# kujason/monopsr

Hardware: AMD Instinct MI355X
Metric: instance-crops/sec (fwd+Chamfer) (higher is better)
Workload: dtype f32; 1 GPU; BASELINE cfg3: batch=256/GPU synthetic 48x48 crops -> ResNet-101 trunk(block3, os4) + squash/map-decoder/xyz + heads fwd, + 1024-pt nn_distance Chamfer fwd/bwd; batch_per_gpu=256, global_batch=256, points=1024, streams_per_gpu=1

## Files before the change

### monopsr_amd/csrc/image_ops.hip

```cpp
#include "common.h"

#pragma clang fp contract(off)

namespace {

template <int V>
struct Vec;
template <>
struct Vec<4> {
    using type = float4;
};
template <>
struct Vec<1> {
    using type = float;
};

__device__ __forceinline__ float4 lerp4(float4 a, float4 b, float t)
{
    return make_float4(a.x + (b.x - a.x) * t, a.y + (b.y - a.y) * t, a.z + (b.z - a.z) * t, a.w + (b.w - a.w) * t);
}
__device__ __forceinline__ float lerp4(float a, float b, float t) { return a + (b - a) * t; }
__device__ __forceinline__ float4 splat(float v, float4) { return make_float4(v, v, v, v); }
__device__ __forceinline__ float splat(float v, float) { return v; }
__device__ __forceinline__ float4 vmax(float4 a, float4 b)
{
    return make_float4(fmaxf(a.x, b.x), fmaxf(a.y, b.y), fmaxf(a.z, b.z), fmaxf(a.w, b.w));
}
__device__ __forceinline__ float vmax(float a, float b) { return fmaxf(a, b); }

template <int V>
__global__ __launch_bounds__(256) void crop_and_resize_kernel(const float *__restrict__ image, int H, int W, int C,
                                                              const float *__restrict__ boxes,
                                                              const int *__restrict__ box_ind, int nimg, int ch,
                                                              int cw, float extrap, float *__restrict__ out,
                                                              long long total)
{
    using T = typename Vec<V>::type;
    const int cv = C / V;
    for (long long i = (long long)blockIdx.x * blockDim.x + threadIdx.x; i < total;
         i += (long long)gridDim.x * blockDim.x) {
        const int c = (int)(i % cv);
        long long r = i / cv;
        const int x = (int)(r % cw);
        r /= cw;
        const int y = (int)(r % ch);
        const int bi = (int)(r / ch);
        const float y1 = boxes[4 * bi], x1 = boxes[4 * bi + 1], y2 = boxes[4 * bi + 2], x2 = boxes[4 * bi + 3];
        const int img = box_ind ? box_ind[bi] : 0;
        T res = splat(extrap, T());
        const float hs = ch > 1 ? (y2 - y1) * (float)(H - 1) / (float)(ch - 1) : 0.f;
        const float ws = cw > 1 ? (x2 - x1) * (float)(W - 1) / (float)(cw - 1) : 0.f;
        const float in_y = ch > 1 ? y1 * (float)(H - 1) + (float)y * hs : 0.5f * (y1 + y2) * (float)(H - 1);
        const float in_x = cw > 1 ? x1 * (float)(W - 1) + (float)x * ws : 0.5f * (x1 + x2) * (float)(W - 1);
        if (img >= 0 && img < nimg && !(in_y < 0.f) && !(in_y > (float)(H - 1)) && !(in_x < 0.f) &&
            !(in_x > (float)(W - 1)) && in_y == in_y && in_x == in_x) {
            const int top = (int)floorf(in_y), bot = (int)ceilf(in_y);
            const int left = (int)floorf(in_x), right = (int)ceilf(in_x);
            const float yl = in_y - (float)top, xl = in_x - (float)left;
            const T *base = reinterpret_cast<const T *>(image + (size_t)img * H * W * C);
            const T tl = base[((size_t)top * W + left) * cv + c], tr = base[((size_t)top * W + right) * cv + c];
            const T bl = base[((size_t)bot * W + left) * cv + c], br = base[((size_t)bot * W + right) * cv + c];
            res = lerp4(lerp4(tl, tr, xl), lerp4(bl, br, xl), yl);
        }
        reinterpret_cast<T *>(out)[i] = res;
    }
}

template <int V>
__global__ __launch_bounds__(256) void resize_bilinear_kernel(const float *__restrict__ in, int H, int W, int C,
                                                              int OH, int OW, float hscale, float wscale,
                                                              float *__restrict__ out, long long total)
{
    using T = typename Vec<V>::type;
    const int cv = C / V;
    for (long long i = (long long)blockIdx.x * blockDim.x + threadIdx.x; i < total;
         i += (long long)gridDim.x * blockDim.x) {
        const int c = (int)(i % cv);
        long long r = i / cv;
        const int ox = (int)(r % OW);
        r /= OW;
        const int oy = (int)(r % OH);
        const int b = (int)(r / OH);
        const float sy = (float)oy * hscale, sx = (float)ox * wscale;
        const int y0 = (int)floorf(sy), x0 = (int)floorf(sx);
        const int y1 = min(y0 + 1, H - 1), x1 = min(x0 + 1, W - 1);
        const float yl = sy - (float)y0, xl = sx - (float)x0;
        const T *base = reinterpret_cast<const T *>(in + (size_t)b * H * W * C);
        const T tl = base[((size_t)y0 * W + x0) * cv + c], tr = base[((size_t)y0 * W + x1) * cv + c];
        const T bl = base[((size_t)y1 * W + x0) * cv + c], br = base[((size_t)y1 * W + x1) * cv + c];
        reinterpret_cast<T *>(out)[i] = lerp4(lerp4(tl, tr, xl), lerp4(bl, br, xl), yl);
    }
}

template <int V>
__global__ __launch_bounds__(256) void resize_bilinear_rows_kernel(const float *__restrict__ in, int H, int W, int C,
                                                                   int OH, int OW, float hscale, float wscale,
                                                                   float *__restrict__ out)
{
    using T = typename Vec<V>::type;
    const unsigned cv = (unsigned)(C / V);
    const unsigned idx = blockIdx.x * 256u + threadIdx.x;
    if (idx >= (unsigned)OW * cv) return;
    const unsigned ox = idx / cv, c = idx - ox * cv;
    const int oy = blockIdx.y, b = blockIdx.z;
    const float sy = (float)oy * hscale, sx = (float)ox * wscale;
    const int y0 = (int)floorf(sy), x0 = (int)floorf(sx);
    const int y1 = min(y0 + 1, H - 1), x1 = min(x0 + 1, W - 1);
    const float yl = sy - (float)y0, xl = sx - (float)x0;
    const T *base = reinterpret_cast<const T *>(in + (size_t)b * H * W * C);
    const T tl = base[((size_t)y0 * W + x0) * cv + c], tr = base[((size_t)y0 * W + x1) * cv + c];
    const T bl = base[((size_t)y1 * W + x0) * cv + c], br = base[((size_t)y1 * W + x1) * cv + c];
    reinterpret_cast<T *>(out)[((size_t)b * OH + oy) * OW * cv + idx] = lerp4(lerp4(tl, tr, xl), lerp4(bl, br, xl), yl);
}

__global__ __launch_bounds__(256) void resize_bilinear_c8out_kernel(const float *__restrict__ in, int H, int W, int C,
                                                                    int OH, int OW, float hscale, float wscale,
                                                                    float *__restrict__ out)
{
    const unsigned planes = (unsigned)C / 8u;
    const unsigned idx = blockIdx.x * 256u + threadIdx.x;
    if (idx >= planes * (unsigned)OW) return;
    const unsigned plane = idx / (unsigned)OW, ox = idx - plane * (unsigned)OW;
    const int oy = blockIdx.y, b = blockIdx.z;
    const float sy = (float)oy * hscale, sx = (float)ox * wscale;
    const int y0 = (int)floorf(sy), x0 = (int)floorf(sx);
    const int y1 = min(y0 + 1, H - 1), x1 = min(x0 + 1, W - 1);
    const float yl = sy - (float)y0, xl = sx - (float)x0;
    const float4 *base = reinterpret_cast<const float4 *>(in + (size_t)b * H * W * C) + plane * 2;
    const size_t cv = (size_t)C / 4;
    float4 *dst = reinterpret_cast<float4 *>(out + ((((size_t)b * planes + plane) * OH + oy) * OW + ox) * 8);
#pragma unroll
    for (int h = 0; h < 2; ++h) {
        const float4 tl = base[((size_t)y0 * W + x0) * cv + h], tr = base[((size_t)y0 * W + x1) * cv + h];
        const float4 bl = base[((size_t)y1 * W + x0) * cv + h], br = base[((size_t)y1 * W + x1) * cv + h];
        dst[h] = lerp4(lerp4(tl, tr, xl), lerp4(bl, br, xl), yl);
    }
}

constexpr int kResizeLdsMaxRows = 16, kResizeLdsIters = 4;
__global__ __launch_bounds__(256) void resize_bilinear_c8out_lds_kernel(const float *__restrict__ in, int H, int W, int C,
                                                                        int OH, int OW, int RO, float hscale,
                                                                        float wscale, float *__restrict__ out)
{
    extern __shared__ __attribute__((aligned(16))) float4 rows[];
    const int plane = blockIdx.x, oy0 = blockIdx.y * RO, b = blockIdx.z;
    const int planes = C / 8;
    const int oy_last = min(oy0 + RO, OH) - 1;
    const int y_lo = (int)floorf((float)oy0 * hscale);
    const int y_hi = min((int)floorf((float)oy_last * hscale) + 1, H - 1);
    const int nrows = y_hi - y_lo + 1;
    const float4 *base = reinterpret_cast<const float4 *>(in + (size_t)b * H * W * C) + plane * 2;
    const size_t cv = (size_t)C / 4;
    for (int i = threadIdx.x; i < nrows * W * 2; i += 256) {
        const int h = i & 1, px = i >> 1;
        const int r = px / W, x = px - r * W;
        rows[i] = base[((size_t)(y_lo + r) * W + x) * cv + h];
    }
    __syncthreads();
    const int rpi = 256 / OW;
    const int r = threadIdx.x / OW, ox = threadIdx.x - r * OW;
    if (r >= rpi) return;
    const float sx = (float)ox * wscale;
    const int x0 = (int)floorf(sx), x1 = min(x0 + 1, W - 1);
    const float xl = sx - (float)x0;
    for (int oy = oy0 + r; oy <= oy_last; oy += rpi) {
        const float sy = (float)oy * hscale;
        const int y0 = (int)floorf(sy), y1 = min(y0 + 1, H - 1);
        const float yl = sy - (float)y0;
        float4 *dst = reinterpret_cast<float4 *>(out + ((((size_t)b * planes + plane) * OH + oy) * OW + ox) * 8);
#pragma unroll
        for (int h = 0; h < 2; ++h) {
            const float4 tl = rows[((y0 - y_lo) * W + x0) * 2 + h], tr = rows[((y0 - y_lo) * W + x1) * 2 + h];
            const float4 bl = rows[((y1 - y_lo) * W + x0) * 2 + h], br = rows[((y1 - y_lo) * W + x1) * 2 + h];
            dst[h] = lerp4(lerp4(tl, tr, xl), lerp4(bl, br, xl), yl);
        }
    }
}

template <int V>
__global__ __launch_bounds__(256) void max_pool_kernel(const float *__restrict__ in, int H, int W, int C, int OH,
                                                       int OW, int k, int s, int pad_top, int pad_left,
                                                       float *__restrict__ out, long long total)
{
    using T = typename Vec<V>::type;
    const int cv = C / V;
    for (long long i = (long long)blockIdx.x * blockDim.x + threadIdx.x; i < total;
         i += (long long)gridDim.x * blockDim.x) {
        const int c = (int)(i % cv);
        long long r = i / cv;
        const int ox = (int)(r % OW);
        r /= OW;
        const int oy = (int)(r % OH);
        const int b = (int)(r / OH);
        const T *base = reinterpret_cast<const T *>(in + (size_t)b * H * W * C);
        T best = splat(-__builtin_inff(), T());
        for (int ky = 0; ky < k; ++ky) {
            const int y = oy * s - pad_top + ky;
            if (y < 0 || y >= H) continue;
            for (int kx = 0; kx < k; ++kx) {
                const int x = ox * s - pad_left + kx;
                if (x < 0 || x >= W) continue;
                best = vmax(best, base[((size_t)y * W + x) * cv + c]);
            }
        }
        reinterpret_cast<T *>(out)[i] = best;
    }
}

__global__ __launch_bounds__(256) void im2col_root_kernel(const float *__restrict__ x, int H, int W, int OH, int OW,
                                                          int kpad, float *__restrict__ cols, long long total)
{
    for (long long i = (long long)blockIdx.x * blockDim.x + threadIdx.x; i < total;
         i += (long long)gridDim.x * blockDim.x) {
        const int j = (int)(i % kpad);
        long long r = i / kpad;
        const int ox = (int)(r % OW);
        r /= OW;
        const int oy = (int)(r % OH);
        const int b = (int)(r / OH);
        float v = 0.f;
        if (j < 147) {
            const int c = j % 3, t = j / 3;
            const int kx = t % 7, ky = t / 7;
            const int yy = oy * 2 + ky - 3, xx = ox * 2 + kx - 3;
            if (yy >= 0 && yy < H && xx >= 0 && xx < W) v = x[(((size_t)b * H + yy) * W + xx) * 3 + c];
        }
        cols[i] = v;
    }
}

__global__ __launch_bounds__(256) void im2col_root_rows_kernel(const float *__restrict__ x, int H, int W, int OW,
                                                               int kpad, float *__restrict__ cols)
{
    const unsigned q4 = (unsigned)kpad / 4u;
    const unsigned idx = blockIdx.x * 256u + threadIdx.x;
    if (idx >= (unsigned)OW * q4) return;
    const unsigned ox = idx / q4, jq = idx - ox * q4;
    const int oy = blockIdx.y, b = blockIdx.z, OH = gridDim.y;
    const float *xb = x + (size_t)b * H * W * 3;
    float v[4];
#pragma unroll
    for (int u = 0; u < 4; ++u) {
        const int j = (int)jq * 4 + u;
        v[u] = 0.f;
        if (j < 147) {
            const int t = j / 3, c = j - 3 * t;
            const int ky = t / 7, kx = t - 7 * ky;
            const int yy = oy * 2 + ky - 3, xx = (int)ox * 2 + kx - 3;
            if (yy >= 0 && yy < H && xx >= 0 && xx < W) v[u] = xb[((size_t)yy * W + xx) * 3 + c];
        }
    }
    reinterpret_cast<float4 *>(cols)[((size_t)b * OH + oy) * OW * q4 + idx] = make_float4(v[0], v[1], v[2], v[3]);
}

inline int grid_for(long long total) { return (int)((total + 255) / 256 < 262144 ? (total + 255) / 256 : 262144); }

inline bool aligned16(const void *p) { return (reinterpret_cast<uintptr_t>(p) & 15) == 0; }

}

extern "C" int mpsr_crop_and_resize(const float *image, int nimg, int H, int W, int C, const float *boxes,
                                    const int *box_ind, int nb, int ch, int cw, float extrapolation_value, float *out,
                                    mpsr_stream_t stream)
{
    MPSR_REQUIRE(nimg > 0 && H > 0 && W > 0 && C > 0 && nb >= 0 && ch > 0 && cw > 0,
                 "crop_and_resize: bad shape (nimg=%d H=%d W=%d C=%d nb=%d crop=%dx%d)", nimg, H, W, C, nb, ch, cw);
    if (nb == 0) return MPSR_OK;
    MPSR_REQUIRE(image && boxes && out, "crop_and_resize: null pointer");
    hipStream_t s = mpsr::as_stream(stream);
    if (C % 4 == 0 && aligned16(image) && aligned16(out)) {
        const long long total = (long long)nb * ch * cw * (C / 4);
        hipLaunchKernelGGL(crop_and_resize_kernel<4>, dim3(grid_for(total)), dim3(256), 0, s, image, H, W, C, boxes,
                           box_ind, nimg, ch, cw, extrapolation_value, out, total);
    } else {
        const long long total = (long long)nb * ch * cw * C;
        hipLaunchKernelGGL(crop_and_resize_kernel<1>, dim3(grid_for(total)), dim3(256), 0, s, image, H, W, C, boxes,
                           box_ind, nimg, ch, cw, extrapolation_value, out, total);
    }
    MPSR_CHECK_LAUNCH("crop_and_resize_kernel");
    return MPSR_OK;
}

extern "C" int mpsr_resize_bilinear(const float *in, int B, int H, int W, int C, int OH, int OW, int align_corners,
                                    float *out, mpsr_stream_t stream)
{
    MPSR_REQUIRE(B >= 0 && H > 0 && W > 0 && C > 0 && OH > 0 && OW > 0, "resize_bilinear: bad shape");
    if (B == 0) return MPSR_OK;
    MPSR_REQUIRE(in && out, "resize_bilinear: null pointer");
    const float hscale = (align_corners && OH > 1) ? (float)(H - 1) / (float)(OH - 1) : (float)H / (float)OH;
    const float wscale = (align_corners && OW > 1) ? (float)(W - 1) / (float)(OW - 1) : (float)W / (float)OW;
    hipStream_t s = mpsr::as_stream(stream);
    if (C % 4 == 0 && aligned16(in) && aligned16(out) && B <= 65535 && OH <= 65535 &&
        (long long)OW * (C / 4) < 0x7fffffffLL) {
        const dim3 grid((unsigned)mpsr::ceil_div(OW * (C / 4), 256), (unsigned)OH, (unsigned)B);
        hipLaunchKernelGGL(resize_bilinear_rows_kernel<4>, grid, dim3(256), 0, s, in, H, W, C, OH, OW, hscale, wscale,
                           out);
    } else if (C % 4 == 0 && aligned16(in) && aligned16(out)) {
        const long long total = (long long)B * OH * OW * (C / 4);
        hipLaunchKernelGGL(resize_bilinear_kernel<4>, dim3(grid_for(total)), dim3(256), 0, s, in, H, W, C, OH, OW,
                           hscale, wscale, out, total);
    } else {
        const long long total = (long long)B * OH * OW * C;
        hipLaunchKernelGGL(resize_bilinear_kernel<1>, dim3(grid_for(total)), dim3(256), 0, s, in, H, W, C, OH, OW,
                           hscale, wscale, out, total);
    }
    MPSR_CHECK_LAUNCH("resize_bilinear_kernel");
    return MPSR_OK;
}

namespace mpsr {
int resize_bilinear_c8(const float *in, int B, int H, int W, int C, int OH, int OW, int align_corners, float *out,
                       hipStream_t s)
{
    MPSR_REQUIRE(B > 0 && H > 0 && W > 0 && C > 0 && C % 8 == 0 && OH > 0 && OW > 0 && B <= 65535 && OH <= 65535 && in &&
                     out && aligned16(in) && aligned16(out),
                 "resize_bilinear_c8: bad arguments");
    const float hscale = (align_corners && OH > 1) ? (float)(H - 1) / (float)(OH - 1) : (float)H / (float)OH;
    const float wscale = (align_corners && OW > 1) ? (float)(W - 1) / (float)(OW - 1) : (float)W / (float)OW;
    if (OW <= 128 && C / 8 <= 65535) {
        int RO = 0, span = 0;
        for (int it = OH >= 40 ? kResizeLdsIters : 1; it >= 1; --it) {
            RO = it * (256 / OW);
            if (RO > OH) RO = OH;
            span = (int)floorf((float)(RO - 1) * hscale) + 3;
            if (span <= kResizeLdsMaxRows) break;
        }
        if (span <= kResizeLdsMaxRows) {
            const dim3 grid((unsigned)(C / 8), (unsigned)ceil_div(OH, RO), (unsigned)B);
            const size_t lds = (size_t)kResizeLdsMaxRows * W * 2 * sizeof(float4);
            if (lds <= 48 * 1024) {
                hipLaunchKernelGGL(resize_bilinear_c8out_lds_kernel, grid, dim3(256), lds, s, in, H, W, C, OH, OW, RO,
                                   hscale, wscale, out);
                MPSR_CHECK_LAUNCH("resize_bilinear_c8out_lds_kernel");
                return MPSR_OK;
            }
        }
    }
    const dim3 grid((unsigned)ceil_div((C / 8) * OW, 256), (unsigned)OH, (unsigned)B);
    hipLaunchKernelGGL(resize_bilinear_c8out_kernel, grid, dim3(256), 0, s, in, H, W, C, OH, OW, hscale, wscale, out);
    MPSR_CHECK_LAUNCH("resize_bilinear_c8out_kernel");
    return MPSR_OK;
}
}

extern "C" int mpsr_max_pool(const float *in, int B, int H, int W, int C, int k, int s_, int pad_same, float *out,
                             mpsr_stream_t stream)
{
    MPSR_REQUIRE(B >= 0 && H > 0 && W > 0 && C > 0 && k > 0 && s_ > 0, "max_pool: bad shape");
    if (B == 0) return MPSR_OK;
    MPSR_REQUIRE(in && out, "max_pool: null pointer");
    int OH, OW, pt = 0, pl = 0;
    if (pad_same) {
        OH = mpsr::ceil_div(H, s_);
        OW = mpsr::ceil_div(W, s_);
        const int th = (OH - 1) * s_ + k - H, tw = (OW - 1) * s_ + k - W;
        pt = (th > 0 ? th : 0) / 2;
        pl = (tw > 0 ? tw : 0) / 2;
    } else {
        MPSR_REQUIRE(H >= k && W >= k, "max_pool: VALID window %d larger than input %dx%d", k, H, W);
        OH = (H - k) / s_ + 1;
        OW = (W - k) / s_ + 1;
    }
    hipStream_t s = mpsr::as_stream(stream);
    if (C % 4 == 0 && aligned16(in) && aligned16(out)) {
        const long long total = (long long)B * OH * OW * (C / 4);
        hipLaunchKernelGGL(max_pool_kernel<4>, dim3(grid_for(total)), dim3(256), 0, s, in, H, W, C, OH, OW, k, s_, pt,
                           pl, out, total);
    } else {
        const long long total = (long long)B * OH * OW * C;
        hipLaunchKernelGGL(max_pool_kernel<1>, dim3(grid_for(total)), dim3(256), 0, s, in, H, W, C, OH, OW, k, s_, pt,
                           pl, out, total);
    }
    MPSR_CHECK_LAUNCH("max_pool_kernel");
    return MPSR_OK;
}

extern "C" int mpsr_im2col_root(const float *x, int B, int H, int W, float *cols, int kpad, mpsr_stream_t stream)
{
    MPSR_REQUIRE(B >= 0 && H >= 1 && W >= 1, "im2col_root: bad shape");
    MPSR_REQUIRE(kpad >= 147 && kpad % 32 == 0, "im2col_root: kpad=%d must be a multiple of 32 and >= 147", kpad);
    if (B == 0) return MPSR_OK;
    MPSR_REQUIRE(x && cols, "im2col_root: null pointer");
    const int OH = (H + 6 - 7) / 2 + 1, OW = (W + 6 - 7) / 2 + 1;
    if (B <= 65535 && OH <= 65535 && aligned16(cols)) {
        const dim3 grid((unsigned)mpsr::ceil_div(OW * (kpad / 4), 256), (unsigned)OH, (unsigned)B);
        hipLaunchKernelGGL(im2col_root_rows_kernel, grid, dim3(256), 0, mpsr::as_stream(stream), x, H, W, OW, kpad,
                           cols);
    } else {
        const long long total = (long long)B * OH * OW * kpad;
        hipLaunchKernelGGL(im2col_root_kernel, dim3(grid_for(total)), dim3(256), 0, mpsr::as_stream(stream), x, H, W,
                           OH, OW, kpad, cols, total);
    }
    MPSR_CHECK_LAUNCH("im2col_root_kernel");
    return MPSR_OK;
}

namespace {

constexpr int kNarrowTile = 16, kNarrowHalo = kNarrowTile + 2, kNarrowCh = 32, kNarrowStride = kNarrowCh + 4;

template <int NOUT>
__global__ __launch_bounds__(256) void conv3x3_narrow_kernel(const float *__restrict__ x, int H, int W, int C,
                                                             const float *__restrict__ w,
                                                             const float *__restrict__ bias, int relu,
                                                             float *__restrict__ y)
{
    __shared__ __attribute__((aligned(16))) float tile[kNarrowHalo * kNarrowHalo * kNarrowStride];
    const int b = blockIdx.z, ty0 = blockIdx.y * kNarrowTile, tx0 = blockIdx.x * kNarrowTile;
    const int tid = threadIdx.x, ly = tid >> 4, lx = tid & 15;
    const float *xb = x + (size_t)b * H * W * C;
    float acc[NOUT];
#pragma unroll
    for (int o = 0; o < NOUT; ++o) acc[o] = 0.f;
    const int K = 9 * C;
    for (int c0 = 0; c0 < C; c0 += kNarrowCh) {
        __syncthreads();
        for (int i = tid; i < kNarrowHalo * kNarrowHalo * (kNarrowCh / 4); i += 256) {
            const int pix = i >> 3, q = i & 7;
            const int py = pix / kNarrowHalo, px = pix - py * kNarrowHalo;
            const int gy = ty0 + py - 1, gx = tx0 + px - 1;
            float4 v = make_float4(0.f, 0.f, 0.f, 0.f);
            if (gy >= 0 && gy < H && gx >= 0 && gx < W && c0 + q * 4 < C)
                v = *reinterpret_cast<const float4 *>(xb + ((size_t)gy * W + gx) * C + c0 + q * 4);
            *reinterpret_cast<float4 *>(&tile[pix * kNarrowStride + q * 4]) = v;
        }
        __syncthreads();
#pragma unroll
        for (int t = 0; t < 9; ++t) {
            const float *src = &tile[((ly + t / 3) * kNarrowHalo + lx + t % 3) * kNarrowStride];
            const float *wt = w + t * C + c0;
#pragma unroll
            for (int q = 0; q < kNarrowCh / 4; ++q) {
                const float4 v = *reinterpret_cast<const float4 *>(src + q * 4);
#pragma unroll
                for (int o = 0; o < NOUT; ++o) {
                    const float *wo = wt + (size_t)o * K + q * 4;
                    acc[o] = fmaf(v.x, wo[0], acc[o]);
                    acc[o] = fmaf(v.y, wo[1], acc[o]);
                    acc[o] = fmaf(v.z, wo[2], acc[o]);
                    acc[o] = fmaf(v.w, wo[3], acc[o]);
                }
            }
        }
    }
    const int oy = ty0 + ly, ox = tx0 + lx;
    if (oy < H && ox < W) {
        float *dst = y + (((size_t)b * H + oy) * W + ox) * NOUT;
#pragma unroll
        for (int o = 0; o < NOUT; ++o) {
            const float v = acc[o] + (bias ? bias[o] : 0.f);
            dst[o] = relu ? fmaxf(v, 0.f) : v;
        }
    }
}

constexpr int kNarrowRows = 8;
using nf32x16 = __attribute__((ext_vector_type(16))) float;

template <int KB, bool IN_C8>
__global__ __launch_bounds__(256) void conv3x3_narrow_mfma_kernel(const float *__restrict__ x, int H, int W,
                                                                  const float *__restrict__ w,
                                                                  const float *__restrict__ bias, int relu, int nout,
                                                                  float *__restrict__ y, unsigned xbytes)
{
    extern __shared__ __attribute__((aligned(16))) float g[];
    constexpr int C = 8 * KB;
    const int b = blockIdx.y, y0 = blockIdx.x * kNarrowRows;
    const int tid = threadIdx.x, lane = tid & 63, wave = __builtin_amdgcn_readfirstlane(tid >> 6);
    const int P = (kNarrowRows + 2) * W;
    float4 bf[KB];
    {
        const int n = lane & 31, t = n / 3, o = n - 3 * t;
        const bool live = n < 9 * 3 && o < nout;
#pragma unroll
        for (int j = 0; j < KB; ++j)
            bf[j] = live ? *reinterpret_cast<const float4 *>(w + (size_t)o * 9 * C + (size_t)t * C + 8 * j + 4 * (lane >> 5))
                         : make_float4(0.f, 0.f, 0.f, 0.f);
    }
    const __amdgpu_buffer_rsrc_t rx = __builtin_amdgcn_make_buffer_rsrc(const_cast<float *>(x), 0, (int)xbytes, 0x00020000);
    const int ntiles = (P + 31) / 32;
    for (int rt = wave; rt < ntiles; rt += 4) {
        const int pix = 32 * rt + (lane & 31);
        const int py = pix / W, gy = y0 - 1 + py;
        const bool ok = pix < P && gy >= 0 && gy < H;
        const unsigned off = !ok ? 0x80000000u
                             : IN_C8 ? (unsigned)((((size_t)b * KB * H + gy) * W + (pix - py * W)) * 8 + 4 * (lane >> 5)) * 4u
                                     : (unsigned)((((size_t)b * H + gy) * W + (pix - py * W)) * C + 4 * (lane >> 5)) * 4u;
        const unsigned kstride = IN_C8 ? (unsigned)H * (unsigned)W * 32u : 32u;
        nf32x16 acc;
#pragma unroll
        for (int e = 0; e < 16; ++e) acc[e] = 0.f;
        float4 a[KB];
#pragma unroll
        for (int j = 0; j < KB; ++j)
            a[j] = __builtin_bit_cast(float4, __builtin_amdgcn_raw_buffer_load_b128(rx, off, (unsigned)j * kstride, 0));
#pragma unroll
        for (int j = 0; j < KB; ++j) {
            acc = __builtin_amdgcn_mfma_f32_32x32x2f32(a[j].x, bf[j].x, acc, 0, 0, 0);
            acc = __builtin_amdgcn_mfma_f32_32x32x2f32(a[j].y, bf[j].y, acc, 0, 0, 0);
            acc = __builtin_amdgcn_mfma_f32_32x32x2f32(a[j].z, bf[j].z, acc, 0, 0, 0);
            acc = __builtin_amdgcn_mfma_f32_32x32x2f32(a[j].w, bf[j].w, acc, 0, 0, 0);
        }
        const int n = lane & 31;
        if (n < 27) {
#pragma unroll
            for (int e = 0; e < 16; ++e) {
                const int pr = 32 * rt + (e & 3) + 8 * (e >> 2) + 4 * (lane >> 5);
                if (pr < P) g[pr * 27 + n] = acc[e];
            }
        }
    }
    __syncthreads();
    const int nrows = min(kNarrowRows, H - y0);
    for (int i = tid; i < nrows * W; i += 256) {
        const int r = i / W, xx = i - r * W;
        float out[3] = {0.f, 0.f, 0.f};
#pragma unroll
        for (int ky = 0; ky < 3; ++ky)
#pragma unroll
            for (int kx = 0; kx < 3; ++kx) {
                const int sx = xx + kx - 1;
                if (sx < 0 || sx >= W) continue;
                const float *src = g + ((r + ky) * W + sx) * 27 + 3 * (ky * 3 + kx);
#pragma unroll
                for (int o = 0; o < 3; ++o) out[o] += src[o];
            }
        float *dst = y + (((size_t)b * H + y0 + r) * W + xx) * nout;
        for (int o = 0; o < nout; ++o) {
            const float v = out[o] + (bias ? bias[o] : 0.f);
            dst[o] = relu ? fmaxf(v, 0.f) : v;
        }
    }
}

}

namespace mpsr {
// ... 58 lines not shown
```

### monopsr_amd/csrc/network.hip

```cpp
#include <atomic>
#include <vector>

#include "common.h"

static std::atomic<int> g_decoder_c8{1};
extern "C" void mpsr_debug_set_decoder_c8(int on) { g_decoder_c8 = on; }
static std::atomic<int> g_decoder_upconv{1};
extern "C" void mpsr_debug_set_decoder_upconv(int on) { g_decoder_upconv = on; }

namespace {

struct Arena {
    char *base;
    size_t size, used = 0;
    bool ok = true;
    Arena(void *p, size_t n) : base(static_cast<char *>(p)), size(n) {}
    float *floats(size_t n)
    {
        const size_t bytes = mpsr::align_up(n * sizeof(float), 256);
        if (used + bytes > size) {
            ok = false;
            return nullptr;
        }
        float *r = reinterpret_cast<float *>(base + used);
// ... 295 lines not shown
                     L[6].cin == c3,
                 "squash_decoder_fwd: layer records are not squash_a, squash_b, conv2_1, conv2_2, conv3_1, conv3_2, xyz");
    Arena ar(workspace, workspace_bytes);
    float *part = ar.floats(Mf * csq), *sq = ar.floats(Mf * csq);
    const size_t r1n = Mh * csq > Mf * 9 * (size_t)c2 ? Mh * csq : Mf * 9 * (size_t)c2;
    const size_t r2n = Mm * c2 > Mh * 9 * (size_t)c3 ? Mm * c2 : Mh * 9 * (size_t)c3;
    float *r1 = ar.floats(r1n), *a = ar.floats(Mh * c2), *b = ar.floats(Mh * c2);
    float *r2 = ar.floats(r2n), *c = ar.floats(Mm * c3);
    float *fm = feat_map ? feat_map : ar.floats(Mm * c3);
    int cwide = csq;
    for (int i = 2; i < n_layers; ++i) cwide = L[i].cout > cwide ? L[i].cout : cwide;
    const size_t skn = mpsr::conv_scratch_floats((long long)Mm, cwide > 512 ? cwide : 512);
    float *sk = ar.floats(skn);
    size_t partn = 0;
    float *partb = nullptr;
    if (ar.ok && mpsr::g_wino4_split.load() != 0 && c2 % 128 == 0 && c3 % 128 == 0 && hh % 4 == 0 && hw % 4 == 0 && mh % 4 == 0 && mw % 4 == 0) {
        const size_t a1 = mpsr::winograd4_split_floats(B, hh, hw, c2), a2 = mpsr::winograd4_split_floats(B, mh, mw, c3);
        partn = (a1 > a2 ? a1 : a2) + 64;
        partb = ar.floats(partn);
        if (!ar.ok) {
            ar.ok = true;
            partb = nullptr;
            partn = 0;
        }
    }
    if (!ar.ok)
        return mpsr::fail(MPSR_ERR_WORKSPACE, "squash_decoder_fwd: workspace %zu bytes too small", workspace_bytes);
    int rc;
    if ((rc = run_layer(blob, L[0], crop_feat, B, fh, fw, nullptr, part, 0, sk, skn, s))) return rc;
    if ((rc = run_layer(blob, L[1], full_feat, B, fh, fw, part, sq, 0, sk, skn, s))) return rc;
    if ((rc = mpsr_max_pool(sq, B, fh, fw, csq, 2, 2, 0, feat_box3d, stream))) return rc;
    if (opts && opts->ready_event) MPSR_CHECK_HIP(hipEventRecord(reinterpret_cast<hipEvent_t>(opts->ready_event), s));
    struct SlotGuard {
        ~SlotGuard() { mpsr::g_filter_cache_slot = mpsr::FilterCacheSlot(); }
    } slot_guard;
    FilterCache cache(opts);
    const DecoderChoice ch = decoder_choice(B, fh, fw, mh, mw, L, blob, feat_map != nullptr, xyz_map != nullptr, sk, skn);
    const bool xyz_c8 = ch.xyz_c8, up1 = ch.up1, up2 = ch.up2, c8 = ch.c8;
    if (c8) {
        auto wino = [&](const mpsr_layer &Lr, const float *x, int H, int W, float *y, int in_c8, int out_c8) {
            cache.offer(blob + Lr.w_off, cache.take(Lr), Lr, (int)(&Lr - L));
            return mpsr::conv3x3_winograd4(x, B, H, W, Lr.cin, blob + Lr.w_off, Lr.b_off >= 0 ? blob + Lr.b_off : nullptr,
                                           Lr.relu, y, Lr.cout, sk, skn, s, in_c8, out_c8, partb, partn);
        };
        auto upconv = [&](const mpsr_layer &Lr, const float *x, int h, int w, int H, int W, float *y, float *z, size_t zn) {
            cache.offer(blob + Lr.w_off, cache.take(Lr), Lr, (int)(&Lr - L));
            return mpsr::conv3x3_upsampled(x, B, h, w, Lr.cin, H, W, 1, blob + Lr.w_off,
                                           Lr.b_off >= 0 ? blob + Lr.b_off : nullptr, Lr.relu, y, Lr.cout, 1, z, zn, sk,
                                           skn, s);
        };
        if (up1) {
            if ((rc = upconv(L[2], sq, fh, fw, hh, hw, a, r1, r1n))) return rc;
        } else {
            if ((rc = mpsr::resize_bilinear_c8(sq, B, fh, fw, csq, hh, hw, 1, r1, s))) return rc;
            if ((rc = wino(L[2], r1, hh, hw, a, 1, 1))) return rc;
        }
        if ((rc = wino(L[3], a, hh, hw, b, 1, 0))) return rc;
        if (up2) {
            if ((rc = upconv(L[4], b, hh, hw, mh, mw, c, r2, r2n))) return rc;
        } else {
            if ((rc = mpsr::resize_bilinear_c8(b, B, hh, hw, c2, mh, mw, 1, r2, s))) return rc;
            if ((rc = wino(L[4], r2, mh, mw, c, 1, 1))) return rc;
        }
        if ((rc = wino(L[5], c, mh, mw, fm, 1, xyz_c8 ? 1 : 0))) return rc;
        if (xyz_map) {
            if (xyz_c8)
                rc = mpsr::conv3x3_narrow(fm, B, mh, mw, L[6].cin, blob + L[6].w_off,
                                          L[6].b_off >= 0 ? blob + L[6].b_off : nullptr, L[6].relu, xyz_map, L[6].cout, s, 1);
            else
                rc = run_layer(blob, L[6], fm, B, mh, mw, nullptr, xyz_map, 1, nullptr, 0, s);
            if (rc) return rc;
        }
        return MPSR_OK;
    }
    auto cached = [&](const mpsr_layer &Lr, const float *x, int H, int W, float *y) {
        cache.offer(blob + Lr.w_off, cache.take(Lr), Lr, (int)(&Lr - L));
        return run_layer(blob, Lr, x, B, H, W, nullptr, y, 0, sk, skn, s);
    };
    auto upconv_nhwc = [&](const mpsr_layer &Lr, const float *x, int h, int w, int H, int W, float *y, float *z, size_t zn) {
        cache.offer(blob + Lr.w_off, cache.take(Lr), Lr, (int)(&Lr - L));
        return mpsr::conv3x3_upsampled(x, B, h, w, Lr.cin, H, W, 1, blob + Lr.w_off,
                                       Lr.b_off >= 0 ? blob + Lr.b_off : nullptr, Lr.relu, y, Lr.cout, 0, z, zn, sk, skn, s);
    };
    if (up1) {
        if ((rc = upconv_nhwc(L[2], sq, fh, fw, hh, hw, a, r1, r1n))) return rc;
    } else {
        if ((rc = mpsr_resize_bilinear(sq, B, fh, fw, csq, hh, hw, 1, r1, stream))) return rc;
        if ((rc = cached(L[2], r1, hh, hw, a))) return rc;
    }
    if ((rc = cached(L[3], a, hh, hw, b))) return rc;
    if (up2) {
        if ((rc = upconv_nhwc(L[4], b, hh, hw, mh, mw, c, r2, r2n))) return rc;
    } else {
        if ((rc = mpsr_resize_bilinear(b, B, hh, hw, c2, mh, mw, 1, r2, stream))) return rc;
        if ((rc = cached(L[4], r2, mh, mw, c))) return rc;
    }
    if ((rc = cached(L[5], c, mh, mw, fm))) return rc;
    if (xyz_map && (rc = run_layer(blob, L[6], fm, B, mh, mw, nullptr, xyz_map, 1, nullptr, 0, s))) return rc;
    return MPSR_OK;
}


namespace {

struct HeadIn {
    const float *boxes, *cam_p, *view, *mean_lwh, *z_off;
    const int *cls;
    const int *cam_idx;
    int n_cams;
    mpsr_head_consts k;
};
__device__ const float kBadCam[12] = {__builtin_nanf(""), __builtin_nanf(""), __builtin_nanf(""), __builtin_nanf(""),
                                      __builtin_nanf(""), __builtin_nanf(""), __builtin_nanf(""), __builtin_nanf(""),
                                      __builtin_nanf(""), __builtin_nanf(""), __builtin_nanf(""), __builtin_nanf("")};
__device__ __forceinline__ const float *cam_of(const HeadIn &in, int b)
{
    if (!in.cam_idx) return in.cam_p;
    const int i = in.cam_idx[b];
    return (i >= 0 && i < in.n_cams) ? in.cam_p + 12 * i : kBadCam;
}

__device__ __forceinline__ float common_feature(const HeadIn &in, int b, int j)
{
    const float *bx = in.boxes + 4 * b;
    const float *cam = cam_of(in, b);
    const float cu = cam[2], cv = cam[6];
    if (j < 4) {
        const float centre = (j & 1) ? cu : cv;
        const float half = ((j & 1) ? in.k.image_w : in.k.image_h) / 2.0f;
        return (bx[j] - centre) / half;
    }
    if (j == 4) return (bx[2] - bx[0]) / in.k.image_h;
    if (j == 5) return in.view[b];
    return (in.cls[b] == j - 6) ? 1.0f : 0.0f;
}

__constant__ float kCamNorm[12] = {1000.f, 1.f, 1000.f, 100.f, 1.f, 1000.f, 1000.f, 1.f, 1.f, 1.f, 1.f, 1.f};

__global__ __launch_bounds__(256) void head_concat_prop_kernel(HeadIn in, const float *__restrict__ imgfc,
                                                               int imgfc_stride, int nfc, int kpad, int B,
                                                               float *__restrict__ out)
{
    const int i = blockIdx.x * blockDim.x + threadIdx.x;
    if (i >= B * kpad) return;
    const int b = i / kpad, col = i - b * kpad;
    const int ncommon = 6 + in.k.num_classes;
    float v = 0.f;
    if (col < nfc) v = imgfc[(size_t)b * imgfc_stride + col];
    else if (col < nfc + ncommon) v = common_feature(in, b, col - nfc);
    else if (col < nfc + ncommon + 12) v = cam_of(in, b)[col - nfc - ncommon] / kCamNorm[col - nfc - ncommon];
    out[i] = v;
}

__global__ __launch_bounds__(256) void head_prop_outputs_kernel(HeadIn in, const float *__restrict__ pout, int B,
                                                                mpsr_head_outputs o, float *__restrict__ prop)
{
    const int b = blockIdx.x * blockDim.x + threadIdx.x;
    if (b >= B) return;
    const int nb = in.k.num_alpha_bins, stride = 3 + 2 * nb;
    const float *p = pout + (size_t)b * stride;
    float lwh[3];
    for (int j = 0; j < 3; ++j) {
        lwh[j] = in.mean_lwh[3 * b + j] + p[j];
        if (o.lwh) o.lwh[3 * b + j] = lwh[j];
        if (o.lwh_offs) o.lwh_offs[3 * b + j] = p[j];
    }
    for (int j = 0; j < nb; ++j) {
        if (o.alpha_bins) o.alpha_bins[(size_t)b * nb + j] = p[3 + j];
        if (o.alpha_regs) o.alpha_regs[(size_t)b * nb + j] = p[3 + nb + j];
    }
    const float *bx = in.boxes + 4 * b;
    const float focal = cam_of(in, b)[0], cv = cam_of(in, b)[6];
    const float z = focal * lwh[2] / (bx[2] - bx[0]) + in.z_off[b];
    const float centre_v = (bx[2] + bx[0]) / 2.0f - cv;
    const float y = centre_v * (z / focal) - in.k.cen_y_class_offset;
    if (o.prop_cen_z) o.prop_cen_z[b] = z;
    prop[2 * b] = y;
    prop[2 * b + 1] = z;
}

__global__ __launch_bounds__(256) void head_concat_reg_kernel(HeadIn in, const float *__restrict__ imgfc,
                                                              int imgfc_stride, int nfc, int kpad, int B,
                                                              const float *__restrict__ pout,
                                                              const float *__restrict__ prop, float *__restrict__ out)
{
    const int i = blockIdx.x * blockDim.x + threadIdx.x;
    if (i >= B * kpad) return;
    const int b = i / kpad, col = i - b * kpad;
    const int ncommon = 6 + in.k.num_classes, nout = 3 + 2 * in.k.num_alpha_bins;
    float v = 0.f;
    if (col < nfc) v = imgfc[(size_t)b * imgfc_stride + nfc + col];
    else if (col < nfc + ncommon) v = common_feature(in, b, col - nfc);
    else if (col < nfc + ncommon + nout) v = pout[(size_t)b * nout + (col - nfc - ncommon)];
    else if (col == nfc + ncommon + nout) v = prop[2 * b] / in.k.cen_y_norm;
    else if (col == nfc + ncommon + nout + 1) v = prop[2 * b + 1] / in.k.max_depth;
    out[i] = v;
}

__global__ __launch_bounds__(256) void head_final_kernel(HeadIn in, const float *__restrict__ rout,
                                                         const float *__restrict__ prop, int B, mpsr_head_outputs o)
{
    const int b = blockIdx.x * blockDim.x + threadIdx.x;
    if (b >= B) return;
    const float yo = rout[2 * b], zo = rout[2 * b + 1];
    const float y = prop[2 * b] + yo, z = prop[2 * b + 1] + zo;
    const float x = z * tanf(in.view[b]) + (-cam_of(in, b)[3] / cam_of(in, b)[0]);
    if (o.cen_y) o.cen_y[b] = y;
    if (o.cen_y_offs) o.cen_y_offs[b] = yo;
    if (o.cen_z) o.cen_z[b] = z;
    if (o.cen_z_offs) o.cen_z_offs[b] = zo;
    if (o.cen_x) o.cen_x[b] = x;
    if (o.centroids) {
        o.centroids[3 * b] = x;
        o.centroids[3 * b + 1] = y;
        o.centroids[3 * b + 2] = z;
    }
}

}

extern "C" size_t mpsr_heads_workspace_bytes(int B, int feat_elems)
{
    if (B <= 0 || feat_elems <= 0) return 0;
    const size_t b = (size_t)B;
    return fbytes(b * 2048) + fbytes(mpsr::conv_scratch_floats(B, 2048)) + 2 * fbytes(b * 1152) + 4 * fbytes(b * 1024) +
           fbytes(b * 64) + fbytes(b * 2) + fbytes(b * 2);
}

extern "C" int mpsr_heads_fwd(const float *feat_box3d, int B, int feat_elems, const float *boxes_2d,
                              const float *cam_p, const float *view_angs, const int *class_idx, const float *mean_lwh,
                              const float *cen_z_offset, const mpsr_head_consts *consts, const float *blob,
                              const mpsr_layer *L, int n_layers, const mpsr_head_outputs *outs, void *workspace,
                              size_t workspace_bytes, mpsr_stream_t stream)
{
    return mpsr_heads_fwd_cams(feat_box3d, B, feat_elems, boxes_2d, cam_p, 1, nullptr, view_angs, class_idx, mean_lwh,
                               cen_z_offset, consts, blob, L, n_layers, outs, workspace, workspace_bytes, stream);
}

extern "C" int mpsr_heads_fwd_cams(const float *feat_box3d, int B, int feat_elems, const float *boxes_2d,
                                   const float *cam_p, int n_cams, const int *cam_index, const float *view_angs,
                                   const int *class_idx, const float *mean_lwh, const float *cen_z_offset,
                                   const mpsr_head_consts *consts, const float *blob, const mpsr_layer *L, int n_layers,
                                   const mpsr_head_outputs *outs, void *workspace, size_t workspace_bytes,
                                   mpsr_stream_t stream)
{
    MPSR_REQUIRE(n_cams >= 1, "heads_fwd: n_cams = %d", n_cams);
    MPSR_REQUIRE(B >= 0 && feat_elems > 0 && feat_elems % 4 == 0, "heads_fwd: bad shape (B=%d feat=%d)", B, feat_elems);
    MPSR_REQUIRE(n_layers == MPSR_HEAD_LAYERS, "heads_fwd: expected %d layer records, got %d", MPSR_HEAD_LAYERS,
                 n_layers);
    if (B == 0) return MPSR_OK;
    MPSR_REQUIRE(feat_box3d && boxes_2d && cam_p && view_angs && class_idx && mean_lwh && cen_z_offset && consts &&
                     blob && L && outs && workspace,
                 "heads_fwd: null pointer");
    const int nfc = L[0].cout / 2;
    const int nb = consts->num_alpha_bins, nc = consts->num_classes;
    const int prop_in = nfc + 6 + nc + 12, reg_in = nfc + 6 + nc + 3 + 2 * nb + 2;
    MPSR_REQUIRE(L[0].cin == feat_elems && L[1].cin >= prop_in && L[1].cin % 4 == 0 && L[3].cout == 3 + 2 * nb &&
                     L[4].cin >= reg_in && L[4].cin % 4 == 0 && L[6].cout == 2 && L[1].cin <= 1152 && L[4].cin <= 1152 &&
                     L[1].cout <= 1024 && L[2].cout <= 1024 && L[4].cout <= 1024 && L[5].cout <= 1024 && nfc <= 1024 &&
                     3 + 2 * nb <= 64,
                 "heads_fwd: layer records do not match the head graph");
    hipStream_t s = mpsr::as_stream(stream);
    Arena ar(workspace, workspace_bytes);
    const size_t b = (size_t)B;
    float *imgfc = ar.floats(b * L[0].cout);
    const size_t skn = mpsr::conv_scratch_floats(B, L[0].cout > 2048 ? L[0].cout : 2048);
    float *skws = ar.floats(skn);
    float *cat_p = ar.floats(b * L[1].cin), *cat_r = ar.floats(b * L[4].cin);
    float *h1 = ar.floats(b * L[1].cout), *h2 = ar.floats(b * L[2].cout);
    float *g1 = ar.floats(b * L[4].cout), *g2 = ar.floats(b * L[5].cout);
    float *pout = ar.floats(b * L[3].cout), *rout = ar.floats(b * 2), *prop = ar.floats(b * 2);
    if (!ar.ok) return mpsr::fail(MPSR_ERR_WORKSPACE, "heads_fwd: workspace %zu bytes too small", workspace_bytes);

    HeadIn in;
    in.boxes = boxes_2d; in.cam_p = cam_p; in.view = view_angs; in.mean_lwh = mean_lwh; in.z_off = cen_z_offset;
    in.cls = class_idx; in.cam_idx = cam_index; in.n_cams = n_cams; in.k = *consts;
    int rc;
    if ((rc = run_layer(blob, L[0], feat_box3d, B, 1, 1, nullptr, imgfc, 0, skws, skn, s))) return rc;
    {
        const int total = B * L[1].cin;
        hipLaunchKernelGGL(head_concat_prop_kernel, dim3(mpsr::ceil_div(total, 256)), dim3(256), 0, s, in, imgfc,
                           L[0].cout, nfc, L[1].cin, B, cat_p);
        MPSR_CHECK_LAUNCH("head_concat_prop_kernel");
    }
    if ((rc = run_layer(blob, L[1], cat_p, B, 1, 1, nullptr, h1, 1, nullptr, 0, s))) return rc;
    if ((rc = run_layer(blob, L[2], h1, B, 1, 1, nullptr, h2, 1, nullptr, 0, s))) return rc;
    if ((rc = run_layer(blob, L[3], h2, B, 1, 1, nullptr, pout, 1, nullptr, 0, s))) return rc;
    hipLaunchKernelGGL(head_prop_outputs_kernel, dim3(mpsr::ceil_div(B, 256)), dim3(256), 0, s, in, pout, B, *outs, prop);
    MPSR_CHECK_LAUNCH("head_prop_outputs_kernel");
    {
        const int total = B * L[4].cin;
        hipLaunchKernelGGL(head_concat_reg_kernel, dim3(mpsr::ceil_div(total, 256)), dim3(256), 0, s, in, imgfc,
                           L[0].cout, nfc, L[4].cin, B, pout, prop, cat_r);
        MPSR_CHECK_LAUNCH("head_concat_reg_kernel");
    }
    if ((rc = run_layer(blob, L[4], cat_r, B, 1, 1, nullptr, g1, 1, nullptr, 0, s))) return rc;
    if ((rc = run_layer(blob, L[5], g1, B, 1, 1, nullptr, g2, 1, nullptr, 0, s))) return rc;
    if ((rc = run_layer(blob, L[6], g2, B, 1, 1, nullptr, rout, 1, nullptr, 0, s))) return rc;
    hipLaunchKernelGGL(head_final_kernel, dim3(mpsr::ceil_div(B, 256)), dim3(256), 0, s, in, rout, prop, B, *outs);
    MPSR_CHECK_LAUNCH("head_final_kernel");
    return MPSR_OK;
}
```

Baseline: 19660 crops/s.

## Specialize stride-2 max pool, add LDS-staged im2col, fuse head prop/concat kernels

Adds a fully unrolled stride-2 max-pool kernel for k=2/3 with 32-bit indexing and NaN propagation, and adds NaN propagation to the generic pool. Adds an im2col root kernel that stages nine input rows in shared memory and emits two output rows per block. It also fuses the head proposal-output and regression-concat kernels into one per-sample block. Together these aim to cut index arithmetic, redundant global loads and one launch, at the cost of extra NaN-check work and more specialized code paths.

Result: no change. 19720 crops/s (median of 6 runs) (+0.3%).

```diff
diff --git a/monopsr_amd/csrc/image_ops.hip b/monopsr_amd/csrc/image_ops.hip
--- a/monopsr_amd/csrc/image_ops.hip
+++ b/monopsr_amd/csrc/image_ops.hip
@@ -27,6 +27,16 @@
     return make_float4(fmaxf(a.x, b.x), fmaxf(a.y, b.y), fmaxf(a.z, b.z), fmaxf(a.w, b.w));
 }
 __device__ __forceinline__ float vmax(float a, float b) { return fmaxf(a, b); }
+__device__ __forceinline__ float nan_of(float n, float v) { return v != v ? v : n; }
+__device__ __forceinline__ float4 nan_of(float4 n, float4 v)
+{
+    return make_float4(nan_of(n.x, v.x), nan_of(n.y, v.y), nan_of(n.z, v.z), nan_of(n.w, v.w));
+}
+__device__ __forceinline__ float with_nan(float best, float n) { return n != n ? n : best; }
+__device__ __forceinline__ float4 with_nan(float4 best, float4 n)
+{
+    return make_float4(with_nan(best.x, n.x), with_nan(best.y, n.y), with_nan(best.z, n.z), with_nan(best.w, n.w));
+}
 
 template <int V>
 __global__ __launch_bounds__(256) void crop_and_resize_kernel(const float *__restrict__ image, int H, int W, int C,
@@ -193,18 +203,54 @@
         const int oy = (int)(r % OH);
         const int b = (int)(r / OH);
         const T *base = reinterpret_cast<const T *>(in + (size_t)b * H * W * C);
-        T best = splat(-__builtin_inff(), T());
+        T best = splat(-__builtin_inff(), T()), nan = splat(0.f, T());
         for (int ky = 0; ky < k; ++ky) {
             const int y = oy * s - pad_top + ky;
             if (y < 0 || y >= H) continue;
             for (int kx = 0; kx < k; ++kx) {
                 const int x = ox * s - pad_left + kx;
                 if (x < 0 || x >= W) continue;
-                best = vmax(best, base[((size_t)y * W + x) * cv + c]);
+                const T v = base[((size_t)y * W + x) * cv + c];
+                best = vmax(best, v);
+                nan = nan_of(nan, v);
             }
         }
-        reinterpret_cast<T *>(out)[i] = best;
-    }
+        reinterpret_cast<T *>(out)[i] = with_nan(best, nan);
+    }
+}
+
+template <int K>
+__global__ __launch_bounds__(256) void max_pool_s2_kernel(const float4 *__restrict__ in, int H, int W, int cv, int OH,
+                                                          int OW, int pad_top, int pad_left, float4 *__restrict__ out,
+                                                          unsigned total)
+{
+    const unsigned i = blockIdx.x * 256u + threadIdx.x;
+    if (i >= total) return;
+    const unsigned c = i % (unsigned)cv;
+    unsigned r = i / (unsigned)cv;
+    const int ox = (int)(r % (unsigned)OW);
+    r /= (unsigned)OW;
+    const int oy = (int)(r % (unsigned)OH);
+    const unsigned b = r / (unsigned)OH;
+    const float4 *base = in + b * (unsigned)(H * W * cv) + c;
+    float4 v[K * K];
+    bool ok[K * K];
+#pragma unroll
+    for (int ky = 0; ky < K; ++ky)
+#pragma unroll
+        for (int kx = 0; kx < K; ++kx) {
+            const int y = oy * 2 - pad_top + ky, x = ox * 2 - pad_left + kx;
+            ok[ky * K + kx] = y >= 0 && y < H && x >= 0 && x < W;
+            v[ky * K + kx] = ok[ky * K + kx] ? base[(unsigned)(y * W + x) * (unsigned)cv] : splat(0.f, float4());
+        }
+    float4 best = splat(-__builtin_inff(), float4()), nan = splat(0.f, float4());
+#pragma unroll
+    for (int t = 0; t < K * K; ++t)
+        if (ok[t]) {
+            best = vmax(best, v[t]);
+            nan = nan_of(nan, v[t]);
+        }
+    out[i] = with_nan(best, nan);
 }
 
 __global__ __launch_bounds__(256) void im2col_root_kernel(const float *__restrict__ x, int H, int W, int OH, int OW,
@@ -251,6 +297,44 @@
         }
     }
     reinterpret_cast<float4 *>(cols)[((size_t)b * OH + oy) * OW * q4 + idx] = make_float4(v[0], v[1], v[2], v[3]);
+}
+
+__global__ __launch_bounds__(256) void im2col_root_pair_kernel(const float *__restrict__ x, int H, int W, int OH, int OW,
+                                                               int kpad, float *__restrict__ cols)
+{
+    extern __shared__ float srows[];
+    const int b = blockIdx.y, oy0 = 2 * blockIdx.x, tid = threadIdx.x;
+    const int w3 = W * 3, rs = w3 + 18;
+    const float *xb = x + (size_t)b * H * w3;
+    for (int r = 0; r < 9; ++r) {
+        const int yy = 2 * oy0 - 3 + r;
+        const bool in = yy >= 0 && yy < H;
+        for (int i = tid; i < rs; i += 256) {
+            const int xi = i - 9;
+            srows[r * rs + i] = (in && xi >= 0 && xi < w3) ? xb[yy * w3 + xi] : 0.f;
+        }
+    }
+    __syncthreads();
+    const int q4 = kpad >> 2, slots = 256 / q4;
+    const int slot = tid / q4, jq = tid - slot * q4;
+    if (slot >= slots) return;
+    int off[4];
+    bool live[4];
+#pragma unroll
+    for (int u = 0; u < 4; ++u) {
+        const int j = jq * 4 + u, ky = j / 21;
+        live[u] = j < 147;
+        off[u] = live[u] ? ky * rs + (j - 21 * ky) : 0;
+    }
+    for (int ro = 0; ro < 2 && oy0 + ro < OH; ++ro) {
+        float4 *dst = reinterpret_cast<float4 *>(cols) + ((size_t)b * OH + oy0 + ro) * OW * q4 + jq;
+        const float *src = srows + 2 * ro * rs;
+        for (int ox = slot; ox < OW; ox += slots) {
+            const float *t = src + 6 * ox;
+            dst[ox * q4] = make_float4(live[0] ? t[off[0]] : 0.f, live[1] ? t[off[1]] : 0.f, live[2] ? t[off[2]] : 0.f,
+                                       live[3] ? t[off[3]] : 0.f);
+        }
+    }
 }
 
 inline int grid_for(long long total) { return (int)((total + 255) / 256 < 262144 ? (total + 255) / 256 : 262144); }
@@ -362,7 +446,17 @@
         OW = (W - k) / s_ + 1;
     }
     hipStream_t s = mpsr::as_stream(stream);
-    if (C % 4 == 0 && aligned16(in) && aligned16(out)) {
+    if (C % 4 == 0 && aligned16(in) && aligned16(out) && s_ == 2 && (k == 2 || k == 3) &&
+        (long long)B * H * W * (C / 4) < 0x7fffffffLL && (long long)B * OH * OW * (C / 4) < 0x7fffffffLL) {
+        const unsigned total = (unsigned)(B * OH * OW * (C / 4));
+        const dim3 grid((total + 255u) / 256u);
+        if (k == 3)
+            hipLaunchKernelGGL(max_pool_s2_kernel<3>, grid, dim3(256), 0, s, reinterpret_cast<const float4 *>(in), H, W,
+                               C / 4, OH, OW, pt, pl, reinterpret_cast<float4 *>(out), total);
+        else
+            hipLaunchKernelGGL(max_pool_s2_kernel<2>, grid, dim3(256), 0, s, reinterpret_cast<const float4 *>(in), H, W,
+                               C / 4, OH, OW, pt, pl, reinterpret_cast<float4 *>(out), total);
+    } else if (C % 4 == 0 && aligned16(in) && aligned16(out)) {
         const long long total = (long long)B * OH * OW * (C / 4);
         hipLaunchKernelGGL(max_pool_kernel<4>, dim3(grid_for(total)), dim3(256), 0, s, in, H, W, C, OH, OW, k, s_, pt,
                            pl, out, total);
@@ -382,7 +476,12 @@
     if (B == 0) return MPSR_OK;
     MPSR_REQUIRE(x && cols, "im2col_root: null pointer");
     const int OH = (H + 6 - 7) / 2 + 1, OW = (W + 6 - 7) / 2 + 1;
-    if (B <= 65535 && OH <= 65535 && aligned16(cols)) {
+    const size_t pair_lds = (size_t)9 * (W + 6) * 3 * sizeof(float);
+    if (B <= 65535 && kpad <= 1024 && pair_lds <= 48 * 1024 && (long long)H * W * 3 < 0x7fffffffLL && aligned16(cols)) {
+        const dim3 grid((unsigned)mpsr::ceil_div(OH, 2), (unsigned)B);
+        hipLaunchKernelGGL(im2col_root_pair_kernel, grid, dim3(256), pair_lds, mpsr::as_stream(stream), x, H, W, OH, OW,
+                           kpad, cols);
+    } else if (B <= 65535 && OH <= 65535 && aligned16(cols)) {
         const dim3 grid((unsigned)mpsr::ceil_div(OW * (kpad / 4), 256), (unsigned)OH, (unsigned)B);
         hipLaunchKernelGGL(im2col_root_rows_kernel, grid, dim3(256), 0, mpsr::as_stream(stream), x, H, W, OW, kpad,
                            cols);
diff --git a/monopsr_amd/csrc/network.hip b/monopsr_amd/csrc/network.hip
--- a/monopsr_amd/csrc/network.hip
+++ b/monopsr_amd/csrc/network.hip
@@ -471,49 +471,46 @@
     out[i] = v;
 }
 
-__global__ __launch_bounds__(256) void head_prop_outputs_kernel(HeadIn in, const float *__restrict__ pout, int B,
-                                                                mpsr_head_outputs o, float *__restrict__ prop)
-{
-    const int b = blockIdx.x * blockDim.x + threadIdx.x;
-    if (b >= B) return;
-    const int nb = in.k.num_alpha_bins, stride = 3 + 2 * nb;
-    const float *p = pout + (size_t)b * stride;
-    float lwh[3];
-    for (int j = 0; j < 3; ++j) {
-        lwh[j] = in.mean_lwh[3 * b + j] + p[j];
-        if (o.lwh) o.lwh[3 * b + j] = lwh[j];
-        if (o.lwh_offs) o.lwh_offs[3 * b + j] = p[j];
-    }
-    for (int j = 0; j < nb; ++j) {
-        if (o.alpha_bins) o.alpha_bins[(size_t)b * nb + j] = p[3 + j];
-        if (o.alpha_regs) o.alpha_regs[(size_t)b * nb + j] = p[3 + nb + j];
-    }
-    const float *bx = in.boxes + 4 * b;
-    const float focal = cam_of(in, b)[0], cv = cam_of(in, b)[6];
-    const float z = focal * lwh[2] / (bx[2] - bx[0]) + in.z_off[b];
-    const float centre_v = (bx[2] + bx[0]) / 2.0f - cv;
-    const float y = centre_v * (z / focal) - in.k.cen_y_class_offset;
-    if (o.prop_cen_z) o.prop_cen_z[b] = z;
-    prop[2 * b] = y;
-    prop[2 * b + 1] = z;
-}
-
-__global__ __launch_bounds__(256) void head_concat_reg_kernel(HeadIn in, const float *__restrict__ imgfc,
-                                                              int imgfc_stride, int nfc, int kpad, int B,
-                                                              const float *__restrict__ pout,
-                                                              const float *__restrict__ prop, float *__restrict__ out)
-{
-    const int i = blockIdx.x * blockDim.x + threadIdx.x;
-    if (i >= B * kpad) return;
-    const int b = i / kpad, col = i - b * kpad;
-    const int ncommon = 6 + in.k.num_classes, nout = 3 + 2 * in.k.num_alpha_bins;
-    float v = 0.f;
-    if (col < nfc) v = imgfc[(size_t)b * imgfc_stride + nfc + col];
-    else if (col < nfc + ncommon) v = common_feature(in, b, col - nfc);
-    else if (col < nfc + ncommon + nout) v = pout[(size_t)b * nout + (col - nfc - ncommon)];
-    else if (col == nfc + ncommon + nout) v = prop[2 * b] / in.k.cen_y_norm;
-    else if (col == nfc + ncommon + nout + 1) v = prop[2 * b + 1] / in.k.max_depth;
-    out[i] = v;
+__global__ __launch_bounds__(256) void head_prop_concat_reg_kernel(HeadIn in, const float *__restrict__ imgfc,
+                                                                   int imgfc_stride, int nfc, int kpad,
+                                                                   const float *__restrict__ pout, mpsr_head_outputs o,
+                                                                   float *__restrict__ prop, float *__restrict__ out)
+{
+    const int b = blockIdx.x;
+    const int nb = in.k.num_alpha_bins, nout = 3 + 2 * nb, ncommon = 6 + in.k.num_classes;
+    const int ycol = nfc + ncommon + nout;
+    float *row = out + (size_t)b * kpad;
+    if (threadIdx.x == 255) {
+        const float *p = pout + (size_t)b * nout;
+        float lwh[3];
+        for (int j = 0; j < 3; ++j) {
+            lwh[j] = in.mean_lwh[3 * b + j] + p[j];
+            if (o.lwh) o.lwh[3 * b + j] = lwh[j];
+            if (o.lwh_offs) o.lwh_offs[3 * b + j] = p[j];
+        }
+        for (int j = 0; j < nb; ++j) {
+            if (o.alpha_bins) o.alpha_bins[(size_t)b * nb + j] = p[3 + j];
+            if (o.alpha_regs) o.alpha_regs[(size_t)b * nb + j] = p[3 + nb + j];
+        }
+        const float *bx = in.boxes + 4 * b;
+        const float focal = cam_of(in, b)[0], cv = cam_of(in, b)[6];
+        const float z = focal * lwh[2] / (bx[2] - bx[0]) + in.z_off[b];
+        const float centre_v = (bx[2] + bx[0]) / 2.0f - cv;
+        const float y = centre_v * (z / focal) - in.k.cen_y_class_offset;
+        if (o.prop_cen_z) o.prop_cen_z[b] = z;
+        prop[2 * b] = y;
+        prop[2 * b + 1] = z;
+        if (ycol < kpad) row[ycol] = y / in.k.cen_y_norm;
+        if (ycol + 1 < kpad) row[ycol + 1] = z / in.k.max_depth;
+    }
+    for (int col = threadIdx.x; col < kpad; col += 256) {
+        if (col == ycol || col == ycol + 1) continue;
+        float v = 0.f;
+        if (col < nfc) v = imgfc[(size_t)b * imgfc_stride + nfc + col];
+        else if (col < nfc + ncommon) v = common_feature(in, b, col - nfc);
+        else if (col < ycol) v = pout[(size_t)b * nout + (col - nfc - ncommon)];
+        row[col] = v;
+    }
 }
 
 __global__ __launch_bounds__(256) void head_final_kernel(HeadIn in, const float *__restrict__ rout,
@@ -605,14 +602,9 @@
     if ((rc = run_layer(blob, L[1], cat_p, B, 1, 1, nullptr, h1, 1, nullptr, 0, s))) return rc;
     if ((rc = run_layer(blob, L[2], h1, B, 1, 1, nullptr, h2, 1, nullptr, 0, s))) return rc;
     if ((rc = run_layer(blob, L[3], h2, B, 1, 1, nullptr, pout, 1, nullptr, 0, s))) return rc;
-    hipLaunchKernelGGL(head_prop_outputs_kernel, dim3(mpsr::ceil_div(B, 256)), dim3(256), 0, s, in, pout, B, *outs, prop);
-    MPSR_CHECK_LAUNCH("head_prop_outputs_kernel");
-    {
-        const int total = B * L[4].cin;
-        hipLaunchKernelGGL(head_concat_reg_kernel, dim3(mpsr::ceil_div(total, 256)), dim3(256), 0, s, in, imgfc,
-                           L[0].cout, nfc, L[4].cin, B, pout, prop, cat_r);
-        MPSR_CHECK_LAUNCH("head_concat_reg_kernel");
-    }
+    hipLaunchKernelGGL(head_prop_concat_reg_kernel, dim3(B), dim3(256), 0, s, in, imgfc, L[0].cout, nfc, L[4].cin, pout,
+                       *outs, prop, cat_r);
+    MPSR_CHECK_LAUNCH("head_prop_concat_reg_kernel");
     if ((rc = run_layer(blob, L[4], cat_r, B, 1, 1, nullptr, g1, 1, nullptr, 0, s))) return rc;
     if ((rc = run_layer(blob, L[5], g1, B, 1, 1, nullptr, g2, 1, nullptr, 0, s))) return rc;
     if ((rc = run_layer(blob, L[6], g2, B, 1, 1, nullptr, rout, 1, nullptr, 0, s))) return rc;
```
